# JuliaMolSim/DFTK.jl

Measured on NVIDIA H100. Metric: hpsi_band_applies_per_s, higher is better.
Workload: dtype f64

## Files before the change

### dftk.jl_b200/csrc/api.cu

```cuda
#include <mutex>
#include "structs.cuh"

using namespace dftk;

static std::string g_last_error;
static std::mutex g_err_mutex;

static int record(dftk_b200_ctx* ctx, int code, const std::string& msg) {
  {
    std::lock_guard<std::mutex> lk(g_err_mutex);
    g_last_error = msg;
  }
  if (ctx) ctx->last_error = msg;
  return code;
}

#define API_BEGIN try {
#define API_END(ctx)                                                        \
  }                                                                         \
  catch (const dftk::Error& e) { return record((ctx), e.code, e.what()); }  \
  catch (const std::exception& e) { return record((ctx), DFTK_B200_EINVAL, e.what()); } \
  catch (...) { return record((ctx), DFTK_B200_EINVAL, "unknown C++ exception"); }      \
  return DFTK_B200_OK;

// ... 316 lines not shown
    kb->d_pl_col0.upload(H.pl_col0.data(), H.pl_col0.size(), s);
    kb->d_cx_s0.upload(H.cx_s0.data(), H.cx_s0.size(), s);
    kb->d_cx_n0.upload(H.cx_n0.data(), H.cx_n0.size(), s);
    kb->d_cx_s1.upload(H.cx_s1.data(), H.cx_s1.size(), s);
    kb->d_cx_n1.upload(H.cx_n1.data(), H.cx_n1.size(), s);
    SphereTablesX& T = kb->T;
    T.nx = H.nx; T.ny = H.ny; T.nz = H.nz; T.n_pw = n_pw; T.n_cols = H.n_cols; T.cnt_max = H.cnt_max;
    T.n_zc = H.n_zc; T.col_start = kb->d_col_start.p; T.col_cnt = kb->d_col_cnt.p;
    T.slot_ix = kb->d_slot_ix.p; T.slot_src = kb->d_slot_src.p; T.zlist = kb->d_zlist.p;
    T.colmap = kb->d_colmap.p;
    T.zc_of = kb->d_zc_of.p;
    T.ranges_ok = H.ranges_ok; T.z_s0 = H.z_s0; T.z_n0 = H.z_n0; T.z_s1 = H.z_s1; T.z_n1 = H.z_n1;
    T.pl_s0 = kb->d_pl_s0.p; T.pl_n0 = kb->d_pl_n0.p; T.pl_s1 = kb->d_pl_s1.p; T.pl_n1 = kb->d_pl_n1.p;
    T.pl_col0 = kb->d_pl_col0.p;
    T.cx_s0 = kb->d_cx_s0.p; T.cx_n0 = kb->d_cx_n0.p; T.cx_s1 = kb->d_cx_s1.p; T.cx_n1 = kb->d_cx_n1.p;
    if (kin) {
      kb->kin.ensure(n_pw);
      CUDA_CHECK(cudaMemcpyAsync(kb->kin.p, kin, n_pw * sizeof(double), cudaMemcpyDefault, s));
      kb->has_kin = true;
    }
    if (n_proj > 0) {
      kb->P.ensure((size_t)n_pw * n_proj);
      CUDA_CHECK(cudaMemcpyAsync(kb->P.p, P, (size_t)n_pw * n_proj * sizeof(cplx), cudaMemcpyDefault, s));
      kb->D_host.resize((size_t)n_proj * n_proj);
      CUDA_CHECK(cudaMemcpy(kb->D_host.data(), D, (size_t)n_proj * n_proj * sizeof(double), cudaMemcpyDefault));
      std::vector<double> dc(2 * (size_t)n_proj * n_proj, 0.0);
      for (size_t i = 0; i < (size_t)n_proj * n_proj; ++i) dc[2 * i] = kb->D_host[i];
      kb->Dc.ensure((size_t)n_proj * n_proj);
      CUDA_CHECK(cudaMemcpyAsync(kb->Dc.p, dc.data(), dc.size() * sizeof(double), cudaMemcpyHostToDevice, s));
      if (n_proj <= 96) {
        kb->PD.ensure((size_t)n_pw * n_proj);
        zgemm(ctx, 0, n_pw, n_proj, n_proj, make_double2(1, 0), kb->P.p, n_pw, kb->Dc.p, n_proj, make_double2(0, 0), kb->PD.p, n_pw);
      }
    }
    CUDA_CHECK(cudaStreamSynchronize(s));
  } catch (...) {
    delete kb;
    throw;
  }
  *out = kb;
  API_END(ctx)
}

int dftk_b200_kblock_destroy(dftk_b200_kblock* kb) {
  delete kb;
  return DFTK_B200_OK;
}

__global__ void k_scale_copy(double* dst, const double* src, double f, int64_t n) {
  int64_t i = (int64_t)blockIdx.x * blockDim.x + threadIdx.x;
  if (i < n) dst[i] = src[i] * f;
}

__global__ void k_scale_transpose_xz(double* __restrict__ dst, const double* __restrict__ src, double f, int nx, int ny, int nz) {
  __shared__ double tile[32][33];
  const int y = blockIdx.z, x0 = blockIdx.x * 32, z0 = blockIdx.y * 32;
  for (int i = threadIdx.y; i < 32; i += blockDim.y) {
    const int z = z0 + i, x = x0 + threadIdx.x;
    if (z < nz && x < nx) tile[i][threadIdx.x] = src[((size_t)z * ny + y) * nx + x];
  }
  __syncthreads();
  for (int i = threadIdx.y; i < 32; i += blockDim.y) {
    const int x = x0 + i, z = z0 + threadIdx.x;
    if (x < nx && z < nz) dst[((size_t)x * ny + y) * nz + z] = tile[threadIdx.x][i] * f;
  }
}
// ... 30 lines not shown
int dftk_b200_grid_set_potential(dftk_b200_grid* grid, int spin, const double* V) {
  dftk_b200_ctx* ctx = grid ? grid->ctx : nullptr;
  API_BEGIN
  REQUIRE(grid && (spin == 0 || spin == 1), "grid_set_potential: bad argument");
  if (!V) {
    grid->has_Vs[spin] = false;
    return DFTK_B200_OK;
  }
  const int64_t N = grid->N;
  const double* d = (const double*)stage_in(ctx, V, N * sizeof(double), ctx->stage_in);
  install_potential(grid, d, grid->Vs[spin], grid->Vts[spin]);
  grid->has_Vs[spin] = true;
  API_END(ctx)
}

int dftk_b200_kblock_trim(dftk_b200_kblock* kb) {
  dftk_b200_ctx* ctx = kb ? kb->grid->ctx : nullptr;
  API_BEGIN
  REQUIRE(kb, "kblock_trim: NULL k-block");
  CUDA_CHECK(cudaStreamSynchronize(ctx->stream));
  kb->lobpcg_ws.release();
  kb->small_ws.release();
  kb->slab_x.release();
  kb->slab_stage.release();
  kb->i8_psi_planes.release();
  kb->i8_psi_exps.release();
  for (int i = 0; i < 8; ++i) {
    kb->i8_pool[i].release();
    kb->i8_epool[i].release();
  }
  kb->W1.release();
  kb->W2.release();
  kb->proj.release();
  API_END(ctx)
}

int dftk_b200_kblock_use_grid_potential(dftk_b200_kblock* kb, int spin) {
  dftk_b200_ctx* ctx = kb ? kb->grid->ctx : nullptr;
  API_BEGIN
  REQUIRE(kb && spin >= -1 && spin <= 1, "kblock_use_grid_potential: bad argument");
  if (spin < 0) {
    kb->grid_V = -1;
    kb->has_V = kb->V.p != nullptr;
    return DFTK_B200_OK;
  }
  REQUIRE(kb->grid->has_Vs[spin], "kblock_use_grid_potential: dftk_b200_grid_set_potential was not called for this spin");
  kb->grid_V = spin;
  kb->has_V = true;
  API_END(ctx)
}

int dftk_b200_fft_sphere_to_real(dftk_b200_kblock* kb, const void* psi, void* out_real, int64_t n_bands,
                                 int normalize) {
  dftk_b200_ctx* ctx = kb ? kb->grid->ctx : nullptr;
  API_BEGIN
  REQUIRE(kb && psi && out_real && n_bands >= 0, "fft_sphere_to_real: bad argument");
  with_staging(ctx, psi, (size_t)kb->n_pw * n_bands * sizeof(cplx), out_real,
               (size_t)kb->grid->N * n_bands * sizeof(cplx), false, [&](const void* i, void* o) {
                 kb_sphere_to_real(kb, (const cplx*)i, (cplx*)o, n_bands, normalize ? kb->grid->ifft_norm : 1.0);
               });
  API_END(ctx)
}

int dftk_b200_fft_real_to_sphere(dftk_b200_kblock* kb, const void* in_real, void* out, int64_t n_bands,
                                 int normalize) {
  dftk_b200_ctx* ctx = kb ? kb->grid->ctx : nullptr;
// ... 37 lines not shown
                                       double* out) {
  int64_t b = (int64_t)blockIdx.x * blockDim.x + threadIdx.x;
  if (b >= nb) return;
  double s = 0.0;
  for (int64_t i = 0; i < np; ++i) {
    cplx a = proj[i + np * b], d = dproj[i + np * b];
    s += a.x * d.x + a.y * d.y;
  }
  out[b] = s;
}

int dftk_b200_band_energies(dftk_b200_kblock* kb, const void* psi, int64_t n_bands, double* ekin_host,
                            double* enl_host) {
  dftk_b200_ctx* ctx = kb ? kb->grid->ctx : nullptr;
  API_BEGIN
  REQUIRE(kb && psi && n_bands >= 0, "band_energies: bad argument");
  if (n_bands == 0) return DFTK_B200_OK;
  const cplx* d = (const cplx*)stage_in(ctx, psi, (size_t)kb->n_pw * n_bands * sizeof(cplx), ctx->stage_in);
  double* sc = ctx->scal.ensure(2 * n_bands + 8);
  if (ekin_host) {
    REQUIRE(kb->has_kin, "band_energies: no kinetic term");
    kin_dots(ctx, d, kb->n_pw, kb->kin.p, kb->n_pw, n_bands, sc);
    CUDA_CHECK(cudaMemcpyAsync(ekin_host, sc, n_bands * sizeof(double), cudaMemcpyDeviceToHost, ctx->stream));
  }
  if (enl_host) {
    if (kb->n_proj == 0) {
      CUDA_CHECK(cudaStreamSynchronize(ctx->stream));
      for (int64_t i = 0; i < n_bands; ++i) enl_host[i] = 0.0;
    } else {
      const int64_t np = kb->n_proj;
      cplx* proj = kb->proj.ensure((size_t)2 * np * n_bands);
      cplx* dproj = proj + (size_t)np * n_bands;
      const cplx one = make_double2(1, 0), zero = make_double2(0, 0);
      zgemm(ctx, 2, np, n_bands, kb->n_pw, one, kb->P.p, kb->n_pw, d, kb->n_pw, zero, proj, np);
      zgemm(ctx, 0, np, n_bands, np, one, kb->Dc.p, np, proj, np, zero, dproj, np);
      LAUNCH(ctx, k_nonlocal_band_energy, (unsigned)((n_bands + 63) / 64), 64, 0, (const cplx*)proj,
             (const cplx*)dproj, np, n_bands, sc + n_bands);
      CUDA_CHECK(cudaMemcpyAsync(enl_host, sc + n_bands, n_bands * sizeof(double), cudaMemcpyDeviceToHost, ctx->stream));
    }
  }
  CUDA_CHECK(cudaStreamSynchronize(ctx->stream));
  API_END(ctx)
}

int dftk_b200_band_energies_multi(int64_t n_blocks, dftk_b200_kblock* const* kbs, const void* const* psi, const int32_t* n_bands,
                                  int64_t ld_out, double* ekin_host, double* enl_host) {
  dftk_b200_ctx* ctx = (n_blocks > 0 && kbs && kbs[0]) ? kbs[0]->grid->ctx : nullptr;
  API_BEGIN
  REQUIRE(n_blocks >= 0 && (n_blocks == 0 || (kbs && psi && n_bands)), "band_energies_multi: bad argument");
  for (int64_t i = 0; i < n_blocks; ++i)
    REQUIRE(kbs[i] && psi[i] && is_device_ptr(psi[i]), "band_energies_multi: orbitals must be device memory");
  band_energies_multi(n_blocks, kbs, (const cplx* const*)psi, (const int*)n_bands, ld_out, ekin_host, enl_host);
  API_END(ctx)
}

int dftk_b200_density_accumulate_multi(int64_t n_blocks, dftk_b200_kblock* const* kbs, const void* const* psi,
                                       const double* occ_w_host, int64_t ld_w, const int32_t* n_bands, double* rho) {
  dftk_b200_ctx* ctx = (n_blocks > 0 && kbs && kbs[0]) ? kbs[0]->grid->ctx : nullptr;
  API_BEGIN
  REQUIRE(n_blocks >= 0 && (n_blocks == 0 || (kbs && psi && n_bands && occ_w_host && rho)), "density_accumulate_multi: bad argument");
  if (n_blocks == 0) return DFTK_B200_OK;
  REQUIRE(is_device_ptr(rho), "density_accumulate_multi: rho must be device memory");
  for (int64_t i = 0; i < n_blocks; ++i)
    REQUIRE(kbs[i] && psi[i] && is_device_ptr(psi[i]) && n_bands[i] >= 0 && n_bands[i] <= ld_w,
            "density_accumulate_multi: bad block / orbitals must be device memory");
  if (!kb_density_accumulate_multi((int)n_blocks, kbs, (const cplx* const*)psi, occ_w_host, ld_w, (const int*)n_bands, rho))
    for (int64_t i = 0; i < n_blocks; ++i)
// ... 224 lines not shown
```

### dftk.jl_b200/csrc/blas.cu

```cuda
#include "structs.cuh"

namespace dftk {

__device__ __forceinline__ void cp_async16(void* smem, const void* gmem, bool pred) {
  unsigned s = (unsigned)__cvta_generic_to_shared(smem);
  int sz = pred ? 16 : 0;
  asm volatile("cp.async.cg.shared.global [%0], [%1], 16, %2;\n" ::"r"(s), "l"(gmem), "r"(sz));
}
__device__ __forceinline__ void cp_async_commit() { asm volatile("cp.async.commit_group;\n" ::); }
template <int N>
__device__ __forceinline__ void cp_async_wait() {
  asm volatile("cp.async.wait_group %0;\n" ::"n"(N));
}
__device__ __forceinline__ void dmma16(double (&c)[4], const double (&a)[8], const double (&b)[4]) {
  asm("mma.sync.aligned.m16n8k16.row.col.f64.f64.f64.f64 {%0,%1,%2,%3}, {%4,%5,%6,%7,%8,%9,%10,%11}, "
      "{%12,%13,%14,%15}, {%0,%1,%2,%3};\n"
      : "+d"(c[0]), "+d"(c[1]), "+d"(c[2]), "+d"(c[3])
      : "d"(a[0]), "d"(a[1]), "d"(a[2]), "d"(a[3]), "d"(a[4]), "d"(a[5]), "d"(a[6]), "d"(a[7]), "d"(b[0]), "d"(b[1]),
        "d"(b[2]), "d"(b[3]));
}
__device__ __forceinline__ double neg(double x) {
  return __hiloint2double(__double2hiint(x) ^ (int)0x80000000, __double2loint(x));
}
__device__ __forceinline__ double2 lds128(const double* p) { return *(const double2*)p; }
// ... 201 lines not shown
        const double* p = bs + (wj + 8 * b + g) * LDK + 16 * ks;
        const double2 v0 = lds128(p), v1 = lds128(p + 2);
        bf[b][0] = v0.x; bf[b][1] = v0.y; bf[b][2] = v1.x; bf[b][3] = v1.y;
      }
#pragma unroll
      for (int a = 0; a < 4; ++a) {
        const double* p = as + 8 * ks * LDA_U + 16 * a;
        const double2 z0 = lds128(p), z1 = lds128(p + LDA_U);
        const double af[8] = {z0.x, z0.y, neg(z0.y), z0.x, z1.x, z1.y, neg(z1.y), z1.x};
#pragma unroll
        for (int b = 0; b < 3; ++b)
          if (a < na && b < nb) dmma16(acc[a][b], af, bf[b]);
      }
    }
  }
  cp_async_wait<0>();
  const bool has_beta = (beta.x != 0.0 || beta.y != 0.0);
#pragma unroll
  for (int a = 0; a < 4; ++a)
#pragma unroll
    for (int b = 0; b < 3; ++b)
#pragma unroll
      for (int e = 0; e < 2; ++e) {
        const int64_t grow = r0 + wr + 8 * a + g;
        const int64_t gj = j0 + wj + 8 * b + 2 * t + e;
        if (grow < Krows && gj < n) {
          cplx o = cmul(alpha, make_double2(acc[a][b][e], acc[a][b][2 + e]));
          if (has_beta) o = cadd(o, cmul(beta, C[grow + ldc * gj]));
          C[grow + ldc * gj] = o;
        }
      }
}

static size_t smem_cn(int st) { return (size_t)st * (GT_M + GT_N) * LDK * sizeof(double); }
static size_t smem_nn(int st) { return (size_t)st * (BKC * LDA_U + UT_N * LDK) * sizeof(double); }

__global__ void k_columnwise_dots(const cplx* __restrict__ A, int64_t lda, const cplx* __restrict__ B,
                                  int64_t ldb, int64_t n_rows, cplx* __restrict__ out) {
  const int64_t col = blockIdx.x;
  const cplx* a = A + lda * col;
  const cplx* b = B + ldb * col;
  double sx = 0.0, sy = 0.0;
  for (int64_t i = threadIdx.x; i < n_rows; i += blockDim.x) {
    cplx x = a[i], y = b[i];
    sx += x.x * y.x + x.y * y.y;
    sy += x.x * y.y - x.y * y.x;
  }
  __shared__ double rx[32], ry[32];
  for (int o = 16; o > 0; o >>= 1) {
    sx += __shfl_down_sync(0xffffffffu, sx, o);
    sy += __shfl_down_sync(0xffffffffu, sy, o);
  }
  if ((threadIdx.x & 31) == 0) {
    rx[threadIdx.x >> 5] = sx;
    ry[threadIdx.x >> 5] = sy;
  }
  __syncthreads();
  if (threadIdx.x < 32) {
    int nw = blockDim.x >> 5;
    sx = threadIdx.x < nw ? rx[threadIdx.x] : 0.0;
    sy = threadIdx.x < nw ? ry[threadIdx.x] : 0.0;
    for (int o = 16; o > 0; o >>= 1) {
      sx += __shfl_down_sync(0xffffffffu, sx, o);
      sy += __shfl_down_sync(0xffffffffu, sy, o);
    }
    if (threadIdx.x == 0) out[col] = make_double2(sx, sy);
  }
}
// ... 11 lines not shown
  for (int o = 16; o > 0; o >>= 1) s += __shfl_down_sync(0xffffffffu, s, o);
  if ((threadIdx.x & 31) == 0) r[threadIdx.x >> 5] = s;
  __syncthreads();
  if (threadIdx.x < 32) {
    int nw = blockDim.x >> 5;
    s = threadIdx.x < nw ? r[threadIdx.x] : 0.0;
    for (int o = 16; o > 0; o >>= 1) s += __shfl_down_sync(0xffffffffu, s, o);
    if (threadIdx.x == 0) out[col] = s;
  }
}

__global__ void k_scale_kin_add(const cplx* __restrict__ psi, cplx* __restrict__ hpsi,
                                const double* __restrict__ kin, int64_t n_rows, int64_t total,
                                int accumulate) {
  int64_t idx = (int64_t)blockIdx.x * blockDim.x + threadIdx.x;
  if (idx >= total) return;
  cplx v = make_double2(0.0, 0.0);
  if (kin) {
    double k = kin[idx % n_rows];
    cplx p = psi[idx];
    v = make_double2(k * p.x, k * p.y);
  }
  if (accumulate) v = cadd(v, hpsi[idx]);
  hpsi[idx] = v;
}

void blas_set_attributes() {
  CUDA_CHECK(cudaFuncSetAttribute(k_zgemm_cn<2>, cudaFuncAttributeMaxDynamicSharedMemorySize, (int)smem_cn(2)));
  CUDA_CHECK(cudaFuncSetAttribute(k_zgemm_nn<2>, cudaFuncAttributeMaxDynamicSharedMemorySize, (int)smem_nn(2)));
  CUDA_CHECK(cudaFuncSetAttribute(k_zgemm_cn<3>, cudaFuncAttributeMaxDynamicSharedMemorySize, (int)smem_cn(3)));
  CUDA_CHECK(cudaFuncSetAttribute(k_zgemm_nn<3>, cudaFuncAttributeMaxDynamicSharedMemorySize, (int)smem_nn(3)));
  CUDA_CHECK(cudaFuncSetAttribute(k_zgemm_cn<4>, cudaFuncAttributeMaxDynamicSharedMemorySize, (int)smem_cn(4)));
  CUDA_CHECK(cudaFuncSetAttribute(k_zgemm_nn<4>, cudaFuncAttributeMaxDynamicSharedMemorySize, (int)smem_nn(4)));
}

void columnwise_dots(dftk_b200_ctx* ctx, const cplx* A, int64_t lda, const cplx* B, int64_t ldb,
                     int64_t n_rows, int64_t n_cols, cplx* out_dev) {
  if (n_cols == 0) return;
  LAUNCH(ctx, k_columnwise_dots, (unsigned)n_cols, 256, 0, A, lda, B, ldb, n_rows, out_dev);
}
void kin_dots(dftk_b200_ctx* ctx, const cplx* X, int64_t ldx, const double* kin, int64_t n_rows,
              int64_t n_cols, double* out_dev) {
  if (n_cols == 0) return;
  LAUNCH(ctx, k_kin_dots, (unsigned)n_cols, 256, 0, X, ldx, kin, n_rows, out_dev);
}
void scale_kin_add(dftk_b200_ctx* ctx, const cplx* psi, cplx* hpsi, const double* kin, int64_t n_rows,
                   int64_t n_cols, int accumulate) {
  int64_t total = n_rows * n_cols;
  if (total == 0) return;
  if (!kin && accumulate) return;
  LAUNCH(ctx, k_scale_kin_add, (unsigned)((total + 255) / 256), 256, 0, psi, hpsi, kin, n_rows, total,
         accumulate);
}

void zgemm(dftk_b200_ctx* ctx, int transA, int64_t m, int64_t n, int64_t k, cplx alpha, const cplx* A,
           int64_t lda, const cplx* B, int64_t ldb, cplx beta, cplx* C, int64_t ldc, bool upper_only) {
  if (m == 0 || n == 0) return;
  REQUIRE(transA == 0 || transA == 2, "zgemm: transA must be 0 (N) or 2 (C)");
  if (ctx->gemm_backend == 1) {
    cuDoubleComplex a = make_cuDoubleComplex(alpha.x, alpha.y), b = make_cuDoubleComplex(beta.x, beta.y);
    CUBLAS_CHECK(cublasZgemm(ctx->cublas, transA == 2 ? CUBLAS_OP_C : CUBLAS_OP_N, CUBLAS_OP_N, (int)m,
                             (int)n, (int)k, &a, (const cuDoubleComplex*)A, (int)lda,
                             (const cuDoubleComplex*)B, (int)ldb, &b, (cuDoubleComplex*)C, (int)ldc));
    ctx->launches++;
    return;
  }
  if ((ctx->gemm_backend == 2 || (ctx->gemm_backend == 4 && k >= ctx->i8_min_rows && m >= 32 && n >= 32)) && transA == 2 && k > 0 && alpha.x == 1.0 && alpha.y == 0.0 && beta.x == 0.0 && beta.y == 0.0) {
    zgemm_i8_cn(ctx, m, n, k, A, lda, B, ldb, C, ldc, ctx->gemm_backend == 4);
    return;
  }
  if (ctx->gemm_backend == 4 && transA == 0 && m >= ctx->i8_min_rows && k >= 32 && n >= 16 && alpha.y == 0.0 && beta.y == 0.0 && !upper_only) {
    const I8Operand opA = i8_prepare(ctx, A, lda, k, m, ctx->i8_tmp_planes, ctx->i8_tmp_exps);
    i8_update(ctx, 1, &opA, B, ldb, n, C, ldc, alpha.x, beta.x);
    return;
  }
  if (ctx->gemm_backend == 2 && transA == 0 && k > 0 && alpha.x == 1.0 && alpha.y == 0.0 && beta.y == 0.0 &&
      (beta.x == 0.0 || beta.x == 1.0) && !upper_only) {
    if (zgemm_i8_nn(ctx, m, n, k, A, lda, B, ldb, C, ldc, beta.x == 1.0)) return;
  }
  if (k == 0) {
    LAUNCH(ctx, k_reduce_partials, (unsigned)((m * n + 255) / 256), 256, 0, (const cplx*)nullptr, 0, m, n,
           alpha, beta, C, ldc);
    return;
  }
  const int st = ctx->gemm_stages;
  if (transA == 2) {
    const int64_t mt = (m + GT_M - 1) / GT_M, nt = (n + GT_N - 1) / GT_N;
    const bool upper = upper_only && m == n;
    int64_t tiles = 0;
    for (int64_t bj = 0; bj < nt; ++bj) tiles += upper ? std::min(mt, ((bj + 1) * GT_N + GT_M - 1) / GT_M) : mt;
    const int64_t slots = ctx->sm_count;
    const int64_t max_split = std::min<int64_t>(64, (k + 8 * BKC - 1) / (8 * BKC));
    int64_t nsplit = 1;
    double best = -1.0;
    for (int64_t sp = 1; sp <= max_split; ++sp) {
      const int64_t total = tiles * sp;
      const double eff = (double)total / (double)(((total + slots - 1) / slots) * slots) - 0.002 * sp;
      if (eff > best) {
        best = eff;
        nsplit = sp;
      }
    }
    int64_t kps = (k + nsplit - 1) / nsplit;
    kps = ((kps + BKC - 1) / BKC) * BKC;
    nsplit = (k + kps - 1) / kps;
    cplx* ws = (cplx*)ctx->gemm_ws.ensure((size_t)nsplit * m * n * sizeof(cplx));
    dim3 grid((unsigned)mt, (unsigned)nt, (unsigned)nsplit);
    const int uo = upper ? 1 : 0;
    if (st == 2) LAUNCH(ctx, k_zgemm_cn<2>, grid, GEMM_THREADS, smem_cn(2), A, lda, B, ldb, ws, m, n, k, kps, uo);
    else if (st == 3) LAUNCH(ctx, k_zgemm_cn<3>, grid, GEMM_THREADS, smem_cn(3), A, lda, B, ldb, ws, m, n, k, kps, uo);
    else LAUNCH(ctx, k_zgemm_cn<4>, grid, GEMM_THREADS, smem_cn(4), A, lda, B, ldb, ws, m, n, k, kps, uo);
    LAUNCH(ctx, k_reduce_partials, (unsigned)((m * n + 255) / 256), 256, 0, (const cplx*)ws, (int)nsplit, m,
           n, alpha, beta, C, ldc);
  } else {
    REQUIRE((m + UT_M - 1) / UT_M <= 65535, "zgemm: more than 4.19M rows are not supported by the update kernel grid");
    dim3 grid((unsigned)((n + UT_N - 1) / UT_N), (unsigned)((m + UT_M - 1) / UT_M));
    const int bu = (upper_only && k == n) ? 1 : 0;
    if (st == 2) LAUNCH(ctx, k_zgemm_nn<2>, grid, GEMM_THREADS, smem_nn(2), A, lda, B, ldb, C, ldc, m, n, k, alpha, beta, bu);
    else if (st == 3) LAUNCH(ctx, k_zgemm_nn<3>, grid, GEMM_THREADS, smem_nn(3), A, lda, B, ldb, C, ldc, m, n, k, alpha, beta, bu);
    else LAUNCH(ctx, k_zgemm_nn<4>, grid, GEMM_THREADS, smem_nn(4), A, lda, B, ldb, C, ldc, m, n, k, alpha, beta, bu);
  }
}

void kb_apply_nonlocal(dftk_b200_kblock* kb, const cplx* psi, cplx* hpsi, int64_t n_bands) {
  if (kb->n_proj == 0 || n_bands == 0) return;
  dftk_b200_ctx* ctx = kb->grid->ctx;
  const int64_t np = kb->n_proj;
  cplx* proj = kb->proj.ensure((size_t)2 * np * n_bands);
  cplx* dproj = proj + (size_t)np * n_bands;
  const cplx one = make_double2(1.0, 0.0), zero = make_double2(0.0, 0.0);
  if (ctx->gemm_backend == 4 && np >= 64 && n_bands >= 32 && kb->n_pw >= ctx->i8_min_rows) {
    if (!kb->i8_Pop.planes) kb->i8_Pop = i8_prepare(ctx, kb->P.p, kb->n_pw, np, kb->n_pw, kb->i8_planes, kb->i8_exps);
    const I8Operand op_psi = i8_prepare(ctx, psi, kb->n_pw, n_bands, kb->n_pw, kb->i8_psi_planes, kb->i8_psi_exps);
    i8_gram(ctx, kb->i8_Pop, op_psi, proj, np, false);
    zgemm(ctx, 0, np, n_bands, np, one, kb->Dc.p, np, proj, np, zero, dproj, np);
    i8_update(ctx, 1, &kb->i8_Pop, dproj, np, n_bands, hpsi, kb->n_pw, 1.0, 1.0);
    return;
  }
  zgemm(ctx, 2, np, n_bands, kb->n_pw, one, kb->P.p, kb->n_pw, psi, kb->n_pw, zero, proj, np);
  zgemm(ctx, 0, np, n_bands, np, one, kb->Dc.p, np, proj, np, zero, dproj, np);
  zgemm(ctx, 0, kb->n_pw, n_bands, np, one, kb->P.p, kb->n_pw, dproj, np, one, hpsi, kb->n_pw);
}

}
```

### dftk.jl_b200/csrc/structs.cuh

```cuda
#pragma once
#include "common.cuh"
#include "fft_reg_fwd.cuh"
#include "fft_plan.h"

namespace dftk {
struct SphereTablesX;
struct RegKernels {
  int A, B, T;
  const void *sphere_to_x, *y_backward, *z_apply, *z_to_cube, *z_from_cube, *z_density, *y_forward, *x_to_sphere;
  const void* z_apply_pipe;
  const void* yz_apply;
  const void *sphere_to_xt, *xt_to_sphere;
  const void *m_sphere_to_x, *m_y_backward, *m_z_apply, *m_y_forward, *m_x_to_sphere, *m_z_density;
};
struct FftMultiItem {
  SphereTablesX T;
  const cplx* psi;
  long long ldpsi;
  cplx *W1, *W2;
  const double* V;
  cplx* out;
  long long ldout;
  const double* kin;
  const double* wts;
// ... 19 lines not shown
  double omega;
  double ifft_norm, fft_norm;
  dftk::FftPlan px, py, pz;
  dftk::DevBuf<double> twx, twy, twz;
  int Lx, Ly, Lz;
  const dftk::RegKernels *rx = nullptr, *ry = nullptr, *rz = nullptr;
  dftk::DevBuf<double> Vs[2];
  dftk::DevBuf<double> Vts[2];
  bool has_Vs[2] = {false, false};
};

struct dftk_b200_kblock {
  dftk_b200_grid* grid;
  int64_t n_pw, n_proj;
  int spin;
  double kweight;
  dftk::SphereTablesHost Th;
  dftk::SphereTablesX T;
  dftk::DevBuf<int> d_col_start, d_col_cnt, d_slot_ix, d_slot_src, d_zlist, d_colmap, d_zc_of, d_pl_s0, d_pl_n0, d_pl_s1, d_pl_n1, d_pl_col0, d_cx_s0, d_cx_n0, d_cx_s1,
      d_cx_n1;
  dftk::DevBuf<double> kin;
  bool has_kin = false;
  dftk::DevBuf<dftk::cplx> P;
  std::vector<double> D_host;
  dftk::DevBuf<dftk::cplx> Dc;
  dftk::DevBuf<signed char> i8_pool[8];
  dftk::DevBuf<int> i8_epool[8];
  dftk::I8Operand i8_Pop;
  dftk::DevBuf<signed char> i8_psi_planes;
  dftk::DevBuf<int> i8_psi_exps;
  dftk::DevBuf<signed char> i8_planes;
  dftk::DevBuf<int> i8_exps;
  dftk::DevBuf<dftk::cplx> PD;
  dftk::DevBuf<double> V;
  bool has_V = false;
  int grid_V = -1;
  const double* Vp() const { return grid_V >= 0 ? grid->Vs[grid_V].p : V.p; }
  dftk::DevBuf<double> Vt;
  const double* Vtp() const { return grid_V >= 0 ? grid->Vts[grid_V].p : Vt.p; }
  dftk::DevBuf<dftk::cplx> W1, W2;
  dftk::DevBuf<dftk::cplx> proj;
  dftk::DevBuf<dftk::cplx> lobpcg_ws;
  dftk::DevBuf<dftk::cplx> small_ws;
  dftk::DevBuf<dftk::cplx> slab_x, slab_stage;
  dftk::DevBuf<double> wts;
  dftk::DevBuf<double> scal;
};

namespace dftk {
int band_chunk_for(dftk_b200_kblock* kb, int64_t n_bands, bool with_W2 = true);
bool grid_yz_fusable(const dftk_b200_grid* g);
void fft_cube_inplace(dftk_b200_grid* g, cplx* data, int sign, int64_t batch);
void kb_sphere_to_planes(dftk_b200_kblock* kb, const cplx* psi, int64_t ldpsi, int nb);
void kb_planes_to_sphere(dftk_b200_kblock* kb, cplx* out, int64_t ldout, int nb, double scale,
                         const double* kin, const cplx* psi, int64_t ldpsi, int accumulate);
void kb_apply_local_kinetic(dftk_b200_kblock* kb, const cplx* psi, cplx* hpsi, int64_t n_bands,
                            bool with_local, bool with_kin, bool accumulate);
bool kb_apply_local_kinetic_multi(int n, dftk_b200_kblock* const* kbs, const cplx* const* psi, cplx* const* hpsi,
                                  const int* n_bands, const void* (*upload)(void* self, const void* host, size_t bytes), void* self);
void kb_sphere_to_real(dftk_b200_kblock* kb, const cplx* psi, cplx* cube, int64_t n_bands, double scale);
void kb_real_to_sphere(dftk_b200_kblock* kb, const cplx* cube, cplx* out, int64_t n_bands, double scale);
void kb_density_accumulate(dftk_b200_kblock* kb, const cplx* psi, const double* occ_w_host,
                           int64_t n_bands, double* rho);
bool kb_density_accumulate_multi(int n, dftk_b200_kblock* const* kbs, const cplx* const* psi, const double* occ_w_host,
                                 int64_t ld_w, const int* n_bands, double* rho);
void fft_set_attributes();
void zgemm(dftk_b200_ctx* ctx, int transA, int64_t m, int64_t n, int64_t k, cplx alpha, const cplx* A,
           int64_t lda, const cplx* B, int64_t ldb, cplx beta, cplx* C, int64_t ldc, bool upper_only = false);
void blas_set_attributes();
void kb_apply_nonlocal(dftk_b200_kblock* kb, const cplx* psi, cplx* hpsi, int64_t n_bands);
void columnwise_dots(dftk_b200_ctx* ctx, const cplx* A, int64_t lda, const cplx* B, int64_t ldb,
                     int64_t n_rows, int64_t n_cols, cplx* out_dev);
void kin_dots(dftk_b200_ctx* ctx, const cplx* X, int64_t ldx, const double* kin, int64_t n_rows,
              int64_t n_cols, double* out_dev);
void scale_kin_add(dftk_b200_ctx* ctx, const cplx* psi, cplx* hpsi, const double* kin, int64_t n_rows,
                   int64_t n_cols, int accumulate);
void xc_evaluate(dftk_b200_ctx* ctx, int mask, int n_spin, bool gga, int64_t N, const double* rho,
                 const double* sigma, double* e, double* vrho, double* vsigma);
void symmetrize_fourier(dftk_b200_grid* g, const cplx* in, cplx* out, int n_sym, const int* invS_host,
                        const double* tau_host);
void zgemm_i8_cn(dftk_b200_ctx* ctx, int64_t m, int64_t n, int64_t k, const cplx* A, int64_t lda, const cplx* B, int64_t ldb,
                 cplx* C, int64_t ldc, bool tensor_cores, const signed char* ra_cached = nullptr, const int* ea_cached = nullptr);
void i8tc2_products(dftk_b200_ctx* ctx, const signed char* ra, const signed char* rb, int64_t m, int64_t n, int64_t ldk,
                    int n_mod, short* part, int* res, bool upper_only);
I8Operand i8_prepare(dftk_b200_ctx* ctx, const cplx* X, int64_t ld, int64_t cols, int64_t k, DevBuf<signed char>& store,
                     DevBuf<int>& estore);
void i8_gram(dftk_b200_ctx* ctx, const I8Operand& A, const I8Operand& B, cplx* C, int64_t ldc, bool upper_only);
void i8_update(dftk_b200_ctx* ctx, int n_blocks, const I8Operand* A, const cplx* B, int64_t ldb, int64_t n, cplx* C, int64_t ldc,
               double alpha, double beta);
void i8tc2_products_nn(dftk_b200_ctx* ctx, int n_blocks, const signed char* const* ra, const int* kcols, const int* k_off,
                       int64_t ldm, const signed char* rb, int64_t ldkb, int64_t m, int64_t n, int n_mod, signed char* resid);
void i8tc2_set_attributes();
bool zgemm_i8_nn(dftk_b200_ctx* ctx, int64_t m, int64_t n, int64_t k, const cplx* A, int64_t lda, const cplx* B, int64_t ldb,
                 cplx* C, int64_t ldc, bool accumulate);
void local_forces(dftk_b200_grid* g, const cplx* w, int n_atoms, const double* pos_host, double* out_host);
void kb_nonlocal_force_rows(dftk_b200_kblock* kb, const cplx* psi, const double* occ_w_host, int64_t n_bands,
                            const double* gpk, double* out_host);
void ewald(dftk_b200_ctx* ctx, const double* lattice_colmajor, int n_atoms, const double* charges, const double* positions,
           double eta, const int* glims, const int* rlims, double* energy_host, double* forces_host);
void structure_factor(dftk_b200_grid* g, int n_atoms, const double* pos_host, const double* coeff_host, cplx* out);
void build_projectors(dftk_b200_ctx* ctx, int64_t n_pw, const double* gpk, int n_atoms, const double* pos_host, int n_rows,
                      const cplx* ff, cplx* P);
int lobpcg_run(dftk_b200_kblock* kb, cplx* X, int64_t M, double tol, int miniter, int maxiter,
// ... 16 lines not shown
```

Baseline: 9800.

## Fold nonlocal projector GEMMs using mirror symmetry of plane-wave sphere

Result: faster. 11100 (median of 6 runs) (+13.3%).

```diff
diff --git a/dftk.jl_b200/csrc/api.cu b/dftk.jl_b200/csrc/api.cu
--- a/dftk.jl_b200/csrc/api.cu
+++ b/dftk.jl_b200/csrc/api.cu
@@ -372,6 +372,7 @@
         kb->PD.ensure((size_t)n_pw * n_proj);
         zgemm(ctx, 0, n_pw, n_proj, n_proj, make_double2(1, 0), kb->P.p, n_pw, kb->Dc.p, n_proj, make_double2(0, 0), kb->PD.p, n_pw);
       }
+      kb_setup_fold(kb, map_h.data());
     }
     CUDA_CHECK(cudaStreamSynchronize(s));
   } catch (...) {
@@ -468,6 +469,7 @@
   kb->W1.release();
   kb->W2.release();
   kb->proj.release();
+  kb->fold_ws.release();
   API_END(ctx)
 }
 
@@ -571,7 +573,7 @@
       cplx* proj = kb->proj.ensure((size_t)2 * np * n_bands);
       cplx* dproj = proj + (size_t)np * n_bands;
       const cplx one = make_double2(1, 0), zero = make_double2(0, 0);
-      zgemm(ctx, 2, np, n_bands, kb->n_pw, one, kb->P.p, kb->n_pw, d, kb->n_pw, zero, proj, np);
+      kb_project(kb, d, n_bands, proj);
       zgemm(ctx, 0, np, n_bands, np, one, kb->Dc.p, np, proj, np, zero, dproj, np);
       LAUNCH(ctx, k_nonlocal_band_energy, (unsigned)((n_bands + 63) / 64), 64, 0, (const cplx*)proj,
              (const cplx*)dproj, np, n_bands, sc + n_bands);
diff --git a/dftk.jl_b200/csrc/blas.cu b/dftk.jl_b200/csrc/blas.cu
--- a/dftk.jl_b200/csrc/blas.cu
+++ b/dftk.jl_b200/csrc/blas.cu
@@ -257,8 +257,231 @@
       }
 }
 
+#define RBK 32
+#define RLDK (2 * RBK + 2)
+#define LDR (RBK + 2)
+__device__ __forceinline__ int bswz(int k) { return k ^ ((k >> 2) & 2); }
+
+template <int STAGES>
+__global__ void __launch_bounds__(GEMM_THREADS, 1)
+k_rgemm_cn(const double* __restrict__ A, int64_t lda, const cplx* __restrict__ B, int64_t ldb,
+           cplx* __restrict__ ws, int64_t m, int64_t n, int64_t K, int64_t k_per_split) {
+  extern __shared__ __align__(16) double smem_d[];
+  double* As = smem_d;
+  double* Bs = smem_d + STAGES * GT_M * LDR;
+  const int tid = threadIdx.x, lane = tid & 31, warp = tid >> 5;
+  const int64_t i0 = (int64_t)blockIdx.x * GT_M, j0 = (int64_t)blockIdx.y * GT_N;
+  const int64_t kb = (int64_t)blockIdx.z * k_per_split;
+  const int64_t ke = min(K, kb + k_per_split);
+  const int nkt = (int)((ke - kb + RBK - 1) / RBK);
+  const int wi = (warp & 1) * 32, wj = (warp >> 1) * 24;
+
+  const int akk = 2 * (tid & 15), acol = tid >> 4;
+  const int lkk = tid & (RBK - 1), lcol = tid >> 5;
+  const double* pA = A + kb + akk + lda * (i0 + acol);
+  const cplx* pB = B + kb + lkk + ldb * (j0 + lcol);
+  unsigned okA = 0, okB = 0;
+#pragma unroll
+  for (int r = 0; r < GT_M / 16; ++r) okA |= (i0 + acol + 16 * r < m) ? (1u << r) : 0u;
+#pragma unroll
+  for (int r = 0; r < GT_N / 8; ++r) okB |= (j0 + lcol + 8 * r < n) ? (1u << r) : 0u;
+  auto load_tile = [&](int kt, int slot) {
+    const int64_t koff = (int64_t)kt * RBK;
+    const bool aok = kb + koff + akk < ke;
+    const bool rowok = kb + koff + lkk < ke;
+    double* da = As + ((size_t)slot * GT_M + acol) * LDR + akk;
+    double* db = Bs + ((size_t)slot * GT_N + lcol) * RLDK + 2 * bswz(lkk);
+#pragma unroll
+    for (int r = 0; r < GT_M / 16; ++r) {
+      bool ok = aok && ((okA >> r) & 1u);
+      cp_async16(da + (size_t)16 * r * LDR, ok ? (pA + koff + (int64_t)16 * r * lda) : A, ok);
+    }
+#pragma unroll
+    for (int r = 0; r < GT_N / 8; ++r) {
+      bool ok = rowok && ((okB >> r) & 1u);
+      cp_async16(db + (size_t)8 * r * RLDK, ok ? (pB + koff + (int64_t)8 * r * ldb) : B, ok);
+    }
+  };
+
+  double cr[2][3][4], ci[2][3][4];
+#pragma unroll
+  for (int a = 0; a < 2; ++a)
+#pragma unroll
+    for (int b = 0; b < 3; ++b)
+#pragma unroll
+      for (int e = 0; e < 4; ++e) cr[a][b][e] = ci[a][b][e] = 0.0;
+
+  for (int s = 0; s < STAGES - 1; ++s) {
+    if (s < nkt) load_tile(s, s);
+    cp_async_commit();
+  }
+  const int g = lane >> 2, t = lane & 3;
+  const int na = mma_tiles(m - i0 - wi, 16, 2), nb = mma_tiles(n - j0 - wj, 8, 3);
+  for (int kt = 0; kt < nkt; ++kt) {
+    cp_async_wait<STAGES - 2>();
+    __syncthreads();
+    {
+      int nxt = kt + STAGES - 1;
+      if (nxt < nkt) load_tile(nxt, nxt % STAGES);
+      cp_async_commit();
+    }
+    const double* as = As + (size_t)(kt % STAGES) * GT_M * LDR + 4 * t;
+    const double* bs = Bs + (size_t)(kt % STAGES) * GT_N * RLDK;
+#pragma unroll
+    for (int ks = 0; ks < RBK / 16; ++ks) {
+    double af[2][8];
+#pragma unroll
+    for (int a = 0; a < 2; ++a) {
+      const double* p = as + (wi + 16 * a + g) * LDR + 16 * ks;
+      const double2 x0 = lds128(p), x1 = lds128(p + 2), y0 = lds128(p + 8 * LDR), y1 = lds128(p + 8 * LDR + 2);
+      af[a][0] = x0.x; af[a][1] = y0.x; af[a][2] = x0.y; af[a][3] = y0.y;
+      af[a][4] = x1.x; af[a][5] = y1.x; af[a][6] = x1.y; af[a][7] = y1.y;
+    }
+#pragma unroll
+    for (int b = 0; b < 3; ++b) {
+      const double* p = bs + (wj + 8 * b + g) * RLDK;
+      double br[4], bi[4];
+#pragma unroll
+      for (int s = 0; s < 4; ++s) {
+        const double2 v = lds128(p + 2 * bswz(16 * ks + 4 * t + s));
+        br[s] = v.x;
+        bi[s] = v.y;
+      }
+#pragma unroll
+      for (int a = 0; a < 2; ++a) {
+        if (a < na && b < nb) {
+          dmma16(cr[a][b], af[a], br);
+          dmma16(ci[a][b], af[a], bi);
+        }
+      }
+    }
+    }
+  }
+  cp_async_wait<0>();
+  cplx* out = ws + (size_t)blockIdx.z * m * n;
+#pragma unroll
+  for (int a = 0; a < 2; ++a)
+#pragma unroll
+    for (int b = 0; b < 3; ++b)
+#pragma unroll
+      for (int e = 0; e < 4; ++e) {
+        int64_t gi = i0 + wi + 16 * a + g + 8 * (e >> 1);
+        int64_t gj = j0 + wj + 8 * b + 2 * t + (e & 1);
+        if (gi < m && gj < n) out[gi + m * gj] = make_double2(cr[a][b][e], ci[a][b][e]);
+      }
+}
+
+#define LDRU (UT_M + 4)
+#define LDBU (2 * RBK + 8)
+template <int STAGES>
+__global__ void __launch_bounds__(GEMM_THREADS, 1)
+k_rgemm_nn(const double* __restrict__ A, int64_t lda, const cplx* __restrict__ B, int64_t ldb,
+           cplx* __restrict__ C, int64_t ldc, int64_t Krows, int64_t n, int64_t m) {
+  extern __shared__ __align__(16) double smem_d[];
+  double* As = smem_d;
+  double* Bs = smem_d + STAGES * RBK * LDRU;
+  const int tid = threadIdx.x, lane = tid & 31, warp = tid >> 5;
+  const int64_t r0 = (int64_t)blockIdx.y * UT_M, j0 = (int64_t)blockIdx.x * UT_N;
+  const int nkt = (int)((m + RBK - 1) / RBK);
+  const int wr = (warp & 1) * 32, wj = (warp >> 1) * 24;
+
+  const int arow = 2 * (tid & 31), aii = tid >> 5;
+  const int bii = tid & (RBK - 1), bcol = tid >> 5;
+  const bool arow_ok = r0 + arow < Krows;
+  const double* pA = A + (r0 + arow) + lda * aii;
+  const cplx* pB = B + bii + ldb * (j0 + bcol);
+  unsigned okB = 0;
+#pragma unroll
+  for (int r = 0; r < UT_N / 8; ++r) okB |= (j0 + bcol + 8 * r < n) ? (1u << r) : 0u;
+  auto load_tile = [&](int kt, int slot) {
+    const int64_t i0 = (int64_t)kt * RBK;
+    double* da = As + ((size_t)slot * RBK + aii) * LDRU + arow;
+    double* db = Bs + ((size_t)slot * UT_N + bcol) * LDBU + 2 * bii;
+#pragma unroll
+    for (int r = 0; r < RBK / 8; ++r) {
+      bool ok = arow_ok && (i0 + aii + 8 * r < m);
+      cp_async16(da + (size_t)8 * r * LDRU, ok ? (pA + (i0 + 8 * r) * lda) : A, ok);
+    }
+    const bool iiok = i0 + bii < m;
+#pragma unroll
+    for (int r = 0; r < UT_N / 8; ++r) {
+      bool ok = iiok && ((okB >> r) & 1u);
+      cp_async16(db + (size_t)8 * r * LDBU, ok ? (pB + i0 + (int64_t)8 * r * ldb) : B, ok);
+    }
+  };
+
+  double ar[2][3][4], ai[2][3][4];
+#pragma unroll
+  for (int a = 0; a < 2; ++a)
+#pragma unroll
+    for (int b = 0; b < 3; ++b)
+#pragma unroll
+      for (int e = 0; e < 4; ++e) ar[a][b][e] = ai[a][b][e] = 0.0;
+
+  for (int s = 0; s < STAGES - 1; ++s) {
+    if (s < nkt) load_tile(s, s);
+    cp_async_commit();
+  }
+  const int g = lane >> 2, t = lane & 3;
+  const int na = mma_tiles(Krows - r0 - wr, 16, 2), nb = mma_tiles(n - j0 - wj, 8, 3);
+  for (int kt = 0; kt < nkt; ++kt) {
+    cp_async_wait<STAGES - 2>();
+    __syncthreads();
+    {
+      int nxt = kt + STAGES - 1;
+      if (nxt < nkt) load_tile(nxt, nxt % STAGES);
+      cp_async_commit();
+    }
+    const double* as = As + (size_t)(kt % STAGES) * RBK * LDRU + t * LDRU + wr + 2 * g;
+    const double* bs = Bs + (size_t)(kt % STAGES) * UT_N * LDBU + 2 * t;
+#pragma unroll
+    for (int ks = 0; ks < RBK / 16; ++ks) {
+    double af[2][8];
+#pragma unroll
+    for (int a = 0; a < 2; ++a)
+#pragma unroll
+      for (int s = 0; s < 4; ++s) {
+        const double2 v = lds128(as + (16 * ks + 4 * s) * LDRU + 16 * a);
+        af[a][2 * s] = v.x;
+        af[a][2 * s + 1] = v.y;
+      }
+#pragma unroll
+    for (int b = 0; b < 3; ++b) {
+      const double* p = bs + (wj + 8 * b + g) * LDBU;
+      double br[4], bi[4];
+#pragma unroll
+      for (int s = 0; s < 4; ++s) {
+        const double2 v = lds128(p + 32 * ks + 8 * s);
+        br[s] = v.x;
+        bi[s] = v.y;
+      }
+#pragma unroll
+      for (int a = 0; a < 2; ++a) {
+        if (a < na && b < nb) {
+          dmma16(ar[a][b], af[a], br);
+          dmma16(ai[a][b], af[a], bi);
+        }
+      }
+    }
+    }
+  }
+  cp_async_wait<0>();
+#pragma unroll
+  for (int a = 0; a < 2; ++a)
+#pragma unroll
+    for (int b = 0; b < 3; ++b)
+#pragma unroll
+      for (int e = 0; e < 4; ++e) {
+        const int64_t row = r0 + wr + 16 * a + 2 * g + (e >> 1);
+        const int64_t gj = j0 + wj + 8 * b + 2 * t + (e & 1);
+        if (row < Krows && gj < n) C[row + ldc * gj] = make_double2(ar[a][b][e], ai[a][b][e]);
+      }
+}
+
 static size_t smem_cn(int st) { return (size_t)st * (GT_M + GT_N) * LDK * sizeof(double); }
 static size_t smem_nn(int st) { return (size_t)st * (BKC * LDA_U + UT_N * LDK) * sizeof(double); }
+static size_t smem_rcn(int st) { return (size_t)st * (GT_M * LDR + GT_N * RLDK) * sizeof(double); }
+static size_t smem_rnn(int st) { return (size_t)st * (RBK * LDRU + UT_N * LDBU) * sizeof(double); }
 
 __global__ void k_columnwise_dots(const cplx* __restrict__ A, int64_t lda, const cplx* __restrict__ B,
                                   int64_t ldb, int64_t n_rows, cplx* __restrict__ out) {
@@ -336,6 +559,10 @@
   CUDA_CHECK(cudaFuncSetAttribute(k_zgemm_nn<3>, cudaFuncAttributeMaxDynamicSharedMemorySize, (int)smem_nn(3)));
   CUDA_CHECK(cudaFuncSetAttribute(k_zgemm_cn<4>, cudaFuncAttributeMaxDynamicSharedMemorySize, (int)smem_cn(4)));
   CUDA_CHECK(cudaFuncSetAttribute(k_zgemm_nn<4>, cudaFuncAttributeMaxDynamicSharedMemorySize, (int)smem_nn(4)));
+  CUDA_CHECK(cudaFuncSetAttribute(k_rgemm_cn<2>, cudaFuncAttributeMaxDynamicSharedMemorySize, (int)smem_rcn(2)));
+  CUDA_CHECK(cudaFuncSetAttribute(k_rgemm_nn<2>, cudaFuncAttributeMaxDynamicSharedMemorySize, (int)smem_rnn(2)));
+  CUDA_CHECK(cudaFuncSetAttribute(k_rgemm_cn<3>, cudaFuncAttributeMaxDynamicSharedMemorySize, (int)smem_rcn(3)));
+  CUDA_CHECK(cudaFuncSetAttribute(k_rgemm_nn<3>, cudaFuncAttributeMaxDynamicSharedMemorySize, (int)smem_rnn(3)));
 }
 
 void columnwise_dots(dftk_b200_ctx* ctx, const cplx* A, int64_t lda, const cplx* B, int64_t ldb,
@@ -355,6 +582,25 @@
   if (!kin && accumulate) return;
   LAUNCH(ctx, k_scale_kin_add, (unsigned)((total + 255) / 256), 256, 0, psi, hpsi, kin, n_rows, total,
          accumulate);
+}
+
+static int64_t gram_splits(const dftk_b200_ctx* ctx, int64_t tiles, int64_t k, int64_t* kps) {
+  const int64_t slots = ctx->sm_count;
+  const int64_t max_split = std::min<int64_t>(64, (k + 8 * BKC - 1) / (8 * BKC));
+  int64_t nsplit = 1;
+  double best = -1.0;
+  for (int64_t sp = 1; sp <= max_split; ++sp) {
+    const int64_t total = tiles * sp;
+    const double eff = (double)total / (double)(((total + slots - 1) / slots) * slots) - 0.002 * sp;
+    if (eff > best) {
+      best = eff;
+      nsplit = sp;
+    }
+  }
+  int64_t len = (k + nsplit - 1) / nsplit;
+  len = ((len + BKC - 1) / BKC) * BKC;
+  *kps = len;
+  return (k + len - 1) / len;
 }
 
 void zgemm(dftk_b200_ctx* ctx, int transA, int64_t m, int64_t n, int64_t k, cplx alpha, const cplx* A,
@@ -393,21 +639,8 @@
     const bool upper = upper_only && m == n;
     int64_t tiles = 0;
     for (int64_t bj = 0; bj < nt; ++bj) tiles += upper ? std::min(mt, ((bj + 1) * GT_N + GT_M - 1) / GT_M) : mt;
-    const int64_t slots = ctx->sm_count;
-    const int64_t max_split = std::min<int64_t>(64, (k + 8 * BKC - 1) / (8 * BKC));
-    int64_t nsplit = 1;
-    double best = -1.0;
-    for (int64_t sp = 1; sp <= max_split; ++sp) {
-      const int64_t total = tiles * sp;
-      const double eff = (double)total / (double)(((total + slots - 1) / slots) * slots) - 0.002 * sp;
-      if (eff > best) {
-        best = eff;
-        nsplit = sp;
-      }
-    }
-    int64_t kps = (k + nsplit - 1) / nsplit;
-    kps = ((kps + BKC - 1) / BKC) * BKC;
-    nsplit = (k + kps - 1) / kps;
+    int64_t kps = 0;
+    const int64_t nsplit = gram_splits(ctx, tiles, k, &kps);
     cplx* ws = (cplx*)ctx->gemm_ws.ensure((size_t)nsplit * m * n * sizeof(cplx));
     dim3 grid((unsigned)mt, (unsigned)nt, (unsigned)nsplit);
     const int uo = upper ? 1 : 0;
@@ -426,8 +659,213 @@
   }
 }
 
+
+bool sphere_mirror(int nx, int ny, int nz, int64_t n_pw, const int64_t* map, std::vector<int>& mir) {
+  const int64_t N = (int64_t)nx * ny * nz;
+  const int n[3] = {nx, ny, nz};
+  std::vector<int> G((size_t)3 * n_pw);
+  int lo[3] = {1 << 30, 1 << 30, 1 << 30}, hi[3] = {-(1 << 30), -(1 << 30), -(1 << 30)};
+  for (int64_t i = 0; i < n_pw; ++i) {
+    int64_t lin = map[i];
+    for (int d = 0; d < 3; ++d) {
+      const int c = (int)(lin % n[d]);
+      lin /= n[d];
+      const int g = c <= (n[d] - 1) / 2 ? c : c - n[d];
+      G[3 * i + d] = g;
+      lo[d] = std::min(lo[d], g);
+      hi[d] = std::max(hi[d], g);
+    }
+  }
+  std::vector<int> slot(N, -1);
+  for (int64_t i = 0; i < n_pw; ++i) slot[map[i]] = (int)i;
+  mir.assign(n_pw, -1);
+  for (int64_t i = 0; i < n_pw; ++i) {
+    int64_t lin = 0;
+    for (int d = 2; d >= 0; --d) {
+      const int g = -G[3 * i + d] + lo[d] + hi[d];
+      lin = lin * n[d] + ((g % n[d]) + n[d]) % n[d];
+    }
+    mir[i] = slot[lin];
+    if (mir[i] < 0) return false;
+  }
+  for (int64_t i = 0; i < n_pw; ++i)
+    if (mir[mir[i]] != i) return false;
+  return true;
+}
+
+__global__ void k_fold_check(const cplx* __restrict__ P, int64_t ldp, const int* __restrict__ hi,
+                             const int* __restrict__ hp, int64_t nh, int64_t np, unsigned long long* __restrict__ out) {
+  double dmax = 0.0, pmax = 0.0;
+  for (int64_t idx = (int64_t)blockIdx.x * blockDim.x + threadIdx.x; idx < nh * np; idx += (int64_t)gridDim.x * blockDim.x) {
+    const int64_t h = idx % nh, j = idx / nh;
+    const cplx a = P[hi[h] + ldp * j], b = P[hp[h] + ldp * j];
+    dmax = fmax(dmax, hypot(b.x - a.x, b.y + a.y));
+    pmax = fmax(pmax, fmax(hypot(a.x, a.y), hypot(b.x, b.y)));
+  }
+  for (int o = 16; o > 0; o >>= 1) {
+    dmax = fmax(dmax, __shfl_down_sync(0xffffffffu, dmax, o));
+    pmax = fmax(pmax, __shfl_down_sync(0xffffffffu, pmax, o));
+  }
+  if ((threadIdx.x & 31) == 0) {
+    atomicMax(out, (unsigned long long)__double_as_longlong(dmax));
+    atomicMax(out + 1, (unsigned long long)__double_as_longlong(pmax));
+  }
+}
+
+__global__ void k_fold_projectors(const cplx* __restrict__ P, int64_t ldp, const int* __restrict__ hi, int64_t nh,
+                                  int64_t np, double* __restrict__ R) {
+  const int64_t idx = (int64_t)blockIdx.x * blockDim.x + threadIdx.x;
+  if (idx >= nh * np) return;
+  const int64_t h = idx % nh, j = idx / nh;
+  const cplx a = P[hi[h] + ldp * j];
+  R[h + 2 * nh * j] = a.x;
+  R[nh + h + 2 * nh * j] = a.y;
+}
+
+__global__ void k_fold(const cplx* __restrict__ psi, int64_t ldpsi, const int* __restrict__ hi,
+                       const int* __restrict__ hp, int64_t nh, int64_t nb, cplx* __restrict__ F, int64_t ldf) {
+  const int64_t idx = (int64_t)blockIdx.x * blockDim.x + threadIdx.x;
+  if (idx >= nh * nb) return;
+  const int64_t h = idx % nh, j = idx / nh;
+  const int i = hi[h], p = hp[h];
+  const cplx a = psi[i + ldpsi * j];
+  cplx s = a, u = make_double2(0.0, 0.0);
+  if (p != i) {
+    const cplx b = psi[p + ldpsi * j];
+    s = cadd(a, b);
+    u = make_double2(a.y - b.y, b.x - a.x);
+  }
+  F[h + ldf * j] = s;
+  F[nh + h + ldf * j] = u;
+}
+
+__global__ void k_unfold_acc(const cplx* __restrict__ Y, int64_t ldy, const int* __restrict__ hi,
+                             const int* __restrict__ hp, int64_t nh, int64_t nb, cplx* __restrict__ hpsi, int64_t ldh) {
+  const int64_t idx = (int64_t)blockIdx.x * blockDim.x + threadIdx.x;
+  if (idx >= nh * nb) return;
+  const int64_t h = idx % nh, j = idx / nh;
+  const int i = hi[h], p = hp[h];
+  const cplx a = Y[h + ldy * j];
+  cplx* o = hpsi + ldh * j;
+  if (p == i) {
+    o[i] = cadd(o[i], a);
+    return;
+  }
+  const cplx b = Y[nh + h + ldy * j];
+  o[i] = cadd(o[i], make_double2(a.x - b.y, a.y + b.x));
+  o[p] = cadd(o[p], make_double2(a.x + b.y, a.y - b.x));
+}
+
+void kb_setup_fold(dftk_b200_kblock* kb, const int64_t* map_h) {
+  kb->n_half = 0;
+  if (kb->n_proj == 0) return;
+  dftk_b200_ctx* ctx = kb->grid->ctx;
+  const dftk_b200_grid* g = kb->grid;
+  std::vector<int> mir;
+  if (!sphere_mirror(g->nx, g->ny, g->nz, kb->n_pw, map_h, mir)) return;
+  std::vector<int> hi, hp;
+  for (int64_t i = 0; i < kb->n_pw; ++i)
+    if (i <= mir[i]) {
+      hi.push_back((int)i);
+      hp.push_back(mir[i]);
+    }
+  const int64_t nh = (int64_t)hi.size(), np = kb->n_proj;
+  cudaStream_t s = ctx->stream;
+  kb->fold_i.upload(hi.data(), nh, s);
+  kb->fold_p.upload(hp.data(), nh, s);
+  unsigned long long* d = (unsigned long long*)ctx->scal.ensure(8);
+  CUDA_CHECK(cudaMemsetAsync(d, 0, 2 * sizeof(unsigned long long), s));
+  LAUNCH(ctx, k_fold_check, (unsigned)(4 * ctx->sm_count), 256, 0, (const cplx*)kb->P.p, kb->n_pw,
+         (const int*)kb->fold_i.p, (const int*)kb->fold_p.p, nh, np, d);
+  unsigned long long r[2];
+  CUDA_CHECK(cudaMemcpyAsync(r, d, sizeof(r), cudaMemcpyDeviceToHost, s));
+  CUDA_CHECK(cudaStreamSynchronize(s));
+  double dev, pmax;
+  std::memcpy(&dev, &r[0], sizeof(double));
+  std::memcpy(&pmax, &r[1], sizeof(double));
+  if (!(dev <= 1e-12 * pmax)) {
+    kb->fold_i.release();
+    kb->fold_p.release();
+    return;
+  }
+  kb->R.ensure((size_t)2 * nh * np);
+  LAUNCH(ctx, k_fold_projectors, (unsigned)((nh * np + 255) / 256), 256, 0, (const cplx*)kb->P.p, kb->n_pw,
+         (const int*)kb->fold_i.p, nh, np, kb->R.p);
+  kb->n_half = nh;
+}
+
+#define FOLD_MAX_COLS 384
+static int64_t fold_chunk(int64_t n_bands) {
+  const int64_t c = (n_bands + FOLD_MAX_COLS - 1) / FOLD_MAX_COLS;
+  return (n_bands + c - 1) / c;
+}
+
+static void rgemm_cn(dftk_b200_ctx* ctx, int64_t m, int64_t n, int64_t K, const double* A, int64_t lda, const cplx* B,
+                     int64_t ldb, cplx* C, int64_t ldc) {
+  const int64_t mt = (m + GT_M - 1) / GT_M, nt = (n + GT_N - 1) / GT_N;
+  int64_t kps = 0;
+  const int64_t nsplit = gram_splits(ctx, mt * nt, K, &kps);
+  cplx* ws = (cplx*)ctx->gemm_ws.ensure((size_t)nsplit * m * n * sizeof(cplx));
+  dim3 grid((unsigned)mt, (unsigned)nt, (unsigned)nsplit);
+  if (ctx->gemm_stages == 2) LAUNCH(ctx, k_rgemm_cn<2>, grid, GEMM_THREADS, smem_rcn(2), A, lda, B, ldb, ws, m, n, K, kps);
+  else LAUNCH(ctx, k_rgemm_cn<3>, grid, GEMM_THREADS, smem_rcn(3), A, lda, B, ldb, ws, m, n, K, kps);
+  LAUNCH(ctx, k_reduce_partials, (unsigned)((m * n + 255) / 256), 256, 0, (const cplx*)ws, (int)nsplit, m, n,
+         make_double2(1.0, 0.0), make_double2(0.0, 0.0), C, ldc);
+}
+
+static void rgemm_nn(dftk_b200_ctx* ctx, int64_t Krows, int64_t n, int64_t m, const double* A, int64_t lda,
+                     const cplx* B, int64_t ldb, cplx* C, int64_t ldc) {
+  REQUIRE((Krows + UT_M - 1) / UT_M <= 65535, "rgemm_nn: more than 4.19M rows are not supported by the update kernel grid");
+  dim3 grid((unsigned)((n + UT_N - 1) / UT_N), (unsigned)((Krows + UT_M - 1) / UT_M));
+  if (ctx->gemm_stages == 2) LAUNCH(ctx, k_rgemm_nn<2>, grid, GEMM_THREADS, smem_rnn(2), A, lda, B, ldb, C, ldc, Krows, n, m);
+  else LAUNCH(ctx, k_rgemm_nn<3>, grid, GEMM_THREADS, smem_rnn(3), A, lda, B, ldb, C, ldc, Krows, n, m);
+}
+
+static bool kb_folds(const dftk_b200_kblock* kb) { return kb->n_half > 0 && kb->grid->ctx->gemm_backend == 0; }
+
+void kb_project(dftk_b200_kblock* kb, const cplx* psi, int64_t n_bands, cplx* proj) {
+  dftk_b200_ctx* ctx = kb->grid->ctx;
+  const int64_t np = kb->n_proj, nh = kb->n_half, kf = 2 * nh;
+  if (!kb_folds(kb)) {
+    zgemm(ctx, 2, np, n_bands, kb->n_pw, make_double2(1, 0), kb->P.p, kb->n_pw, psi, kb->n_pw, make_double2(0, 0), proj, np);
+    return;
+  }
+  const int64_t nc = fold_chunk(n_bands);
+  cplx* F = kb->fold_ws.ensure((size_t)kf * nc);
+  for (int64_t j0 = 0; j0 < n_bands; j0 += nc) {
+    const int64_t w = std::min(nc, n_bands - j0);
+    LAUNCH(ctx, k_fold, (unsigned)((nh * w + 255) / 256), 256, 0, psi + kb->n_pw * j0, kb->n_pw,
+           (const int*)kb->fold_i.p, (const int*)kb->fold_p.p, nh, w, F, kf);
+    rgemm_cn(ctx, np, w, kf, kb->R.p, kf, F, kf, proj + np * j0, np);
+  }
+}
+
+static void kb_apply_nonlocal_folded(dftk_b200_kblock* kb, const cplx* psi, cplx* hpsi, int64_t n_bands) {
+  dftk_b200_ctx* ctx = kb->grid->ctx;
+  const int64_t np = kb->n_proj, nh = kb->n_half, kf = 2 * nh;
+  const int64_t nc = fold_chunk(n_bands);
+  cplx* F = kb->fold_ws.ensure((size_t)kf * nc);
+  cplx* proj = kb->proj.ensure((size_t)2 * np * nc);
+  cplx* dproj = proj + (size_t)np * nc;
+  for (int64_t j0 = 0; j0 < n_bands; j0 += nc) {
+    const int64_t w = std::min(nc, n_bands - j0);
+    const unsigned blocks = (unsigned)((nh * w + 255) / 256);
+    LAUNCH(ctx, k_fold, blocks, 256, 0, psi + kb->n_pw * j0, kb->n_pw, (const int*)kb->fold_i.p,
+           (const int*)kb->fold_p.p, nh, w, F, kf);
+    rgemm_cn(ctx, np, w, kf, kb->R.p, kf, F, kf, proj, np);
+    zgemm(ctx, 0, np, w, np, make_double2(1, 0), kb->Dc.p, np, proj, np, make_double2(0, 0), dproj, np);
+    rgemm_nn(ctx, kf, w, np, kb->R.p, kf, dproj, np, F, kf);
+    LAUNCH(ctx, k_unfold_acc, blocks, 256, 0, (const cplx*)F, kf, (const int*)kb->fold_i.p, (const int*)kb->fold_p.p,
+           nh, w, hpsi + kb->n_pw * j0, kb->n_pw);
+  }
+}
+
 void kb_apply_nonlocal(dftk_b200_kblock* kb, const cplx* psi, cplx* hpsi, int64_t n_bands) {
   if (kb->n_proj == 0 || n_bands == 0) return;
+  if (kb_folds(kb)) {
+    kb_apply_nonlocal_folded(kb, psi, hpsi, n_bands);
+    return;
+  }
   dftk_b200_ctx* ctx = kb->grid->ctx;
   const int64_t np = kb->n_proj;
   cplx* proj = kb->proj.ensure((size_t)2 * np * n_bands);
diff --git a/dftk.jl_b200/csrc/structs.cuh b/dftk.jl_b200/csrc/structs.cuh
--- a/dftk.jl_b200/csrc/structs.cuh
+++ b/dftk.jl_b200/csrc/structs.cuh
@@ -75,6 +75,10 @@
   dftk::DevBuf<signed char> i8_planes;
   dftk::DevBuf<int> i8_exps;
   dftk::DevBuf<dftk::cplx> PD;
+  int64_t n_half = 0;
+  dftk::DevBuf<int> fold_i, fold_p;
+  dftk::DevBuf<double> R;
+  dftk::DevBuf<dftk::cplx> fold_ws;
   dftk::DevBuf<double> V;
   bool has_V = false;
   int grid_V = -1;
@@ -112,6 +116,9 @@
            int64_t lda, const cplx* B, int64_t ldb, cplx beta, cplx* C, int64_t ldc, bool upper_only = false);
 void blas_set_attributes();
 void kb_apply_nonlocal(dftk_b200_kblock* kb, const cplx* psi, cplx* hpsi, int64_t n_bands);
+void kb_project(dftk_b200_kblock* kb, const cplx* psi, int64_t n_bands, cplx* proj);
+bool sphere_mirror(int nx, int ny, int nz, int64_t n_pw, const int64_t* map, std::vector<int>& mir);
+void kb_setup_fold(dftk_b200_kblock* kb, const int64_t* map_h);
 void columnwise_dots(dftk_b200_ctx* ctx, const cplx* A, int64_t lda, const cplx* B, int64_t ldb,
                      int64_t n_rows, int64_t n_cols, cplx* out_dev);
 void kin_dots(dftk_b200_ctx* ctx, const cplx* X, int64_t ldx, const double* kin, int64_t n_rows,
```
